# MircoWerner/VkRadixSort

Measured on AMD Instinct MI355X. Metric: Gkeys/s sorting 10^8 uint32 at 1/2/4/8 MI355X; % of HBM roofline, higher is better.
Workload: dtype u32

## Files before the change

vkradixsort_amd/csrc/vrs_device.hpp:

```cpp
#pragma once
#include "vrs_kernels.h"

#include <hip/hip_ext.h>

#include <type_traits>

#define VRS_LAUNCH(kernel, grid, block, stream, ev, ...)                                                        \
    do {                                                                                                        \
        if ((ev).start != nullptr || (ev).stop != nullptr)                                                      \
            hipExtLaunchKernelGGL(kernel, grid, block, 0, stream, (ev).start, (ev).stop, 0, __VA_ARGS__);       \
        else                                                                                                    \
            hipLaunchKernelGGL(kernel, grid, block, 0, stream, __VA_ARGS__);                                    \
    } while (0)

#ifndef VRS_MARK
#define VRS_MARK(i)
#define VRS_MARK_FLUSH(...)
#endif
namespace vrs {

constexpr size_t kStreamInBytes = size_t(128) << 20;

constexpr int kDtUnroll = 8;
constexpr int kLbItems = 16;
// ... 94 lines not shown
    for (int o = 1; o < 64; o <<= 1) {
        const uint32_t t = __shfl_up(incl, o);
        if (lane >= static_cast<uint32_t>(o)) incl += t;
    }
    if (lane == 63u) s_tmp[wave] = incl;
    __syncthreads();
    uint32_t base = 0;
#pragma unroll
    for (int j = 0; j < kWaves; ++j) base += (static_cast<uint32_t>(j) < wave) ? s_tmp[j] : 0u;
    return base + incl - v;
}

constexpr int RANK_BALLOT = 0;
constexpr int RANK_ATOMIC = 1;

template <typename K, int ITEMS, int WAVES, bool PAIRS = false>
struct ChunkSmem {
    K keys[ITEMS * WAVES * 64];
    uint32_t vals[PAIRS ? ITEMS * WAVES * 64 : 1];
    uint32_t whist[WAVES][kBins];
    uint32_t gbase[kBins];
    uint32_t scan_tmp[WAVES];
    uint32_t lb_gave_up;
};

__device__ __forceinline__ uint64_t match_any_digit(uint32_t d) {
    uint32_t lo = ~0u, hi = ~0u;
#pragma unroll
    for (int b = 0; b < 8; ++b) {
        const uint32_t m = static_cast<uint32_t>(__builtin_amdgcn_sbfe(static_cast<int>(d), b, 1));
        const uint64_t B = __builtin_amdgcn_uicmp(m, 0u, 33 );
        lo = __builtin_amdgcn_bitop3_b32(m, lo, static_cast<uint32_t>(B), 0x84);
        hi = __builtin_amdgcn_bitop3_b32(m, hi, static_cast<uint32_t>(B >> 32), 0x84);
    }
    return (static_cast<uint64_t>(hi) << 32) | lo;
}

template <int WAVES>
__device__ __forceinline__ uint32_t block_exclusive_scan_w(uint32_t v, uint32_t *s_tmp, uint32_t lane,
                                                           uint32_t wave) {
    uint32_t incl = v;
#pragma unroll
    for (int o = 1; o < 64; o <<= 1) {
        const uint32_t t = __shfl_up(incl, o);
        if (lane >= static_cast<uint32_t>(o)) incl += t;
    }
    if (lane == 63u) s_tmp[wave] = incl;
    __syncthreads();
    uint32_t base = 0;
#pragma unroll
    for (int j = 0; j < WAVES; ++j) base += (static_cast<uint32_t>(j) < wave) ? s_tmp[j] : 0u;
    return base + incl - v;
}

constexpr uint32_t kLbInclusive = 1u << 28, kLbValue = (1u << 28) - 1u, kLbTagShift = 29;

__device__ __forceinline__ uint32_t lb_load(const uint32_t *p) {
    return __hip_atomic_load(p, __ATOMIC_RELAXED, __HIP_MEMORY_SCOPE_AGENT);
}
__device__ __forceinline__ void lb_store_through(uint32_t *p, uint32_t v) {
    __hip_atomic_store(p, v, __ATOMIC_RELAXED, __HIP_MEMORY_SCOPE_AGENT);
}
__device__ __forceinline__ void lb_store_l2(uint32_t *p, uint32_t v) {
    __hip_atomic_store(p, v, __ATOMIC_RELAXED, __HIP_MEMORY_SCOPE_WORKGROUP);
}

struct NoLookback {
// ... 141 lines not shown
        }
        if constexpr (PAIRS) {
#pragma unroll
            for (int i = 0; i < ITEMS; ++i) {
                const uint32_t idx = seg + i * 64;
                val[i] = vin[FULL ? idx : (idx < valid ? idx : valid - 1u)];
            }
        }
    }
}
template <typename K, int ITEMS, typename DG>
__device__ __forceinline__ void chunk_pad(K (&key)[ITEMS], uint32_t valid, const DG &dg) {
    const uint32_t seg = (threadIdx.x >> 6) * (ITEMS * 64) + (threadIdx.x & 63u);
#pragma unroll
    for (int i = 0; i < ITEMS; ++i) key[i] = seg + i * 64 < valid ? key[i] : dg.template pad<K>();
}

template <typename K, int ITEMS, int WAVES, bool PAIRS, int RANK, bool FULL, typename DG, typename LB = NoLookback>
__device__ __forceinline__ void scatter_chunk_loaded(ChunkSmem<K, ITEMS, WAVES, PAIRS> &sm, K (&key)[ITEMS], uint32_t (&val)[PAIRS ? ITEMS : 1], K *kout,
                                                     uint32_t *vout, uint32_t valid, const DG &dg, uint32_t &run_off, const LB lb = {}) {
    constexpr uint32_t THREADS = WAVES * 64;
    const uint32_t tid = threadIdx.x;
    const uint32_t lane = tid & 63u;
    const uint32_t wave = tid >> 6;

    {
        uint32_t *z = &sm.whist[0][0];
#pragma unroll
        for (int v = 0; v < 4; ++v) z[v * THREADS + tid] = 0;
        if constexpr (LB::kEnabled) {
// ... 137 lines not shown

    if constexpr (PAIRS) {
#pragma unroll
        for (int i = 0; i < ITEMS; ++i) val[i] = sm.vals[i * THREADS + tid];
        if constexpr (LB::kPool) {
            lb.template store_values<ITEMS, THREADS, FULL>(val, dst, vout, valid);
        } else {
#pragma unroll
            for (int i = 0; i < ITEMS; ++i) {
                if (FULL || i * THREADS + tid < valid) vout[dst[i]] = val[i];
            }
        }
    }
}

template <typename K, int ITEMS, int WAVES, bool PAIRS, int RANK, bool FULL, typename DG, typename LB = NoLookback, typename SRC = NoPieces>
__device__ __forceinline__ void scatter_chunk(ChunkSmem<K, ITEMS, WAVES, PAIRS> &sm, const K *kin,
                                              const uint32_t *vin, K *kout, uint32_t *vout,
                                              uint32_t valid, const DG &dg, uint32_t &run_off, const LB lb = {},
                                              const SRC src = {}, bool stream_in = false) {
    VRS_MARK(0);
    K key[ITEMS];
    uint32_t val[PAIRS ? ITEMS : 1];
    if constexpr (SRC::kEnabled) {
        const uint32_t seg = (threadIdx.x >> 6) * (ITEMS * 64) + (threadIdx.x & 63u);
        uint32_t vs[ITEMS];
#pragma unroll
        for (int i = 0; i < ITEMS; ++i) vs[i] = src.first_slot;
#pragma unroll 1
        for (uint32_t p = src.p0; p < src.p1; ++p) {
            const uint32_t lo = __builtin_amdgcn_readlane(src.lo, p), len = __builtin_amdgcn_readlane(src.len, p), vd = __builtin_amdgcn_readlane(src.slot, p);
#pragma unroll
            for (int i = 0; i < ITEMS; ++i) {
                const uint32_t idx = seg + i * 64;
                vs[i] = idx - lo < len ? vd + (idx - lo) : vs[i];
            }
        }
#pragma unroll
        for (int i = 0; i < ITEMS; ++i) {
            const K k = *src.at(vs[i]);
            key[i] = (FULL || seg + i * 64 < valid) ? k : dg.template pad<K>();
        }
        if constexpr (PAIRS) {
#pragma unroll
            for (int i = 0; i < ITEMS; ++i) val[i] = *src.val_at(vs[i]);
        }
    } else {
        chunk_load<K, ITEMS, PAIRS, FULL>(kin, vin, valid, stream_in, key, val);
        if constexpr (!FULL) chunk_pad(key, valid, dg);
    }
    scatter_chunk_loaded<K, ITEMS, WAVES, PAIRS, RANK, FULL, DG, LB>(sm, key, val, kout, vout, valid, dg, run_off, lb);
}

constexpr uint32_t kMsdBits = 14, kMsdBuckets = 1u << kMsdBits;
constexpr uint32_t kMsdMinShift = 13, kMsdMaxShift = 18;
constexpr uint32_t kMsdProbeWord = kMsdBuckets + 8u * 256u, kMsdOverWord = kMsdProbeWord + 1u;
constexpr uint32_t kMsdSubBits = kMsdBits - 8, kMsdSub = 1u << kMsdSubBits;

struct BitsDigit {
    uint32_t shift, mask, base;
    __device__ __forceinline__ uint32_t operator()(uint32_t key) const { return ((key - base) >> shift) & mask; }
// ... 7 lines not shown
```

vkradixsort_amd/csrc/vrs_local_sort.hpp:

```cpp
#pragma once
#include "vrs_device.hpp"

namespace vrs {

constexpr int kLeanRow = 512 + 64;
constexpr int kLeanMaxVec = 7;
template <bool STREAM>
__device__ __forceinline__ void store_sorted(uint4 *p, const uint4 &q) {
    if constexpr (STREAM) {
        typedef uint32_t u32x4 __attribute__((ext_vector_type(4)));
        const u32x4 v = {q.x, q.y, q.z, q.w};
        __builtin_nontemporal_store(v, reinterpret_cast<u32x4 *>(p));
    } else {
        *p = q;
    }
}

__device__ __forceinline__ void rows_in_order() { __builtin_amdgcn_sched_barrier(0); }
template <int STRIDE, int VEC>
__device__ __forceinline__ void load_rows(uint32_t (&k)[4 * VEC], const uint32_t *src, uint32_t words, uint32_t t) {
    const uint32_t nvec = (words + 3u) / 4u;
#pragma unroll
    for (int j = 0; j < VEC; ++j) {
        uint32_t v = j * STRIDE + t;
        if (j == VEC - 1) v = v < nvec ? v : nvec - 1u;
        const uint4 q = reinterpret_cast<const uint4 *>(src)[v];
        if (j + 1 < VEC) rows_in_order();
        k[4 * j] = q.x;
        k[4 * j + 1] = q.y;
        k[4 * j + 2] = q.z;
        k[4 * j + 3] = q.w;
    }
}

__device__ __forceinline__ uint32_t wave_inclusive_sum(uint32_t x) {
    x += __builtin_amdgcn_update_dpp(0u, x, 0x111, 0xf, 0xf, false);
    x += __builtin_amdgcn_update_dpp(0u, x, 0x112, 0xf, 0xf, false);
    x += __builtin_amdgcn_update_dpp(0u, x, 0x114, 0xf, 0xf, false);
    x += __builtin_amdgcn_update_dpp(0u, x, 0x118, 0xf, 0xf, false);
    x += __builtin_amdgcn_update_dpp(0u, x, 0x142, 0xa, 0xf, false);
    x += __builtin_amdgcn_update_dpp(0u, x, 0x143, 0xc, 0xf, false);
    return x;
}

__device__ __forceinline__ void pinned(uint32_t &x) { asm volatile("" : "+v"(x)); }

template <int WAVES>
__device__ __forceinline__ uint32_t waves_before(const uint32_t *s_tmp, uint32_t wave) {
    static_assert(WAVES % 4 == 0, "whole 16-byte vectors");
    uint4 t[WAVES / 4];
#pragma unroll
    for (int g = 0; g < WAVES / 4; ++g) t[g] = reinterpret_cast<const uint4 *>(s_tmp)[g];
    uint32_t sum = 0;
#pragma unroll
    for (int g = 0; g < WAVES / 4; ++g) {
        sum += (4u * g + 0u < wave) ? t[g].x : 0u;
        sum += (4u * g + 1u < wave) ? t[g].y : 0u;
        sum += (4u * g + 2u < wave) ? t[g].z : 0u;
        sum += (4u * g + 3u < wave) ? t[g].w : 0u;
    }
    return sum;
}

template <int THREADS, int VEC, bool GUARD, bool STREAM = false, bool ALIGNED_IN = false>
__device__ __forceinline__ void lean_sort_body(uint32_t (&k)[4 * VEC], uint32_t *abase, uint32_t mis, uint32_t n, uint32_t *s_keys,
                                               uint32_t *s_hist2, uint32_t *s_tmp, bool guard1, bool guard2, uint32_t mis_in) {
    constexpr int WAVES = THREADS / 64, ITEMS = 4 * VEC, PER = 512 / THREADS;
    const uint32_t tid = threadIdx.x, lane = tid & 63u, wave = tid >> 6;
    const uint32_t end = mis + n;
    const uint32_t nvec = (end + 3u) / 4u;
    uint32_t rank[ITEMS];
    uint32_t *s_hist = s_hist2 + WAVES * kLeanRow;
#pragma unroll
    for (int j = 0; j < VEC; ++j)
#pragma unroll
        for (int c = 0; c < 4; ++c) {
            uint32_t a = (k[4 * j + c] << 2) & 0x7FCu;
// ... 504 lines not shown
```

vkradixsort_amd/csrc/vrs_msd_pool.hip:

```cpp
#include "vrs_local_sort.hpp"

#include <algorithm>
#include <cmath>

namespace vrs {

namespace {

constexpr uint32_t kPoolMinShift = 13, kPoolMaxShift = 18;
constexpr float kPoolSigmas = 6.0f;

__global__ __launch_bounds__(256) void pool_sample_kernel(const uint32_t *__restrict__ keys, uint32_t n, uint32_t key_base,
                                                          PoolStreams ps, PoolPlan *__restrict__ pool, uint32_t top_bits) {
    constexpr int kPerWave = kPoolSampleTiles / 4;
    constexpr int kLoads = kPoolSampleKeys / 64;
    __shared__ uint32_t s_hist[2][256];
    __shared__ uint32_t s_or;
    const uint32_t tid = threadIdx.x, lane = tid & 63u, wave = tid >> 6;
    s_hist[0][tid] = 0;
    s_hist[1][tid] = 0;
    if (tid == 0) s_or = 0;
    const uint32_t t0 = blockIdx.x * kPoolSampleTiles;
    const uint32_t s0 = t0 / ps.tiles_per_stream;
    uint32_t k[kPerWave][kLoads];
// ... 104 lines not shown
    static constexpr bool kEnabled = true;
    static constexpr bool kReserves = true;
    static constexpr bool kPool = true;
    bool foreign = false;
    uint32_t recounted = 0;
    int index = 0;
    const void *stream_keys = nullptr;
    uint32_t done = 0;
    uint32_t seed = 0;
    uint32_t *cursor = nullptr;
    const uint32_t *region = nullptr;
    uint32_t pad_keys = 0;
    uint32_t n_virt = 0;
    uint32_t *overflow = nullptr;
    uint32_t overflow_last = 0;
    uint32_t *gbase2 = nullptr, *split = nullptr, *flags = nullptr;
    uint32_t *fail_word = nullptr;
    mutable uint32_t reserved = 0, cnt = 0, rb = 0, rc = 0, ob = 0, oc = 0;
    mutable bool reserved_yet = false;

    __device__ __forceinline__ void publish(uint32_t v) const {
        if (reserved_yet) return;
        reserved_yet = true;
        cnt = v - pad_keys;
        if (cnt) reserved = __hip_atomic_fetch_add(cursor, cnt, __ATOMIC_RELAXED, __HIP_MEMORY_SCOPE_WORKGROUP);
    }
    __device__ __forceinline__ void load_region() {
        rb = region[0];
        rc = region[8 * 256];
        ob = region[16 * 256];
        oc = region[24 * 256];
// ... 9 lines not shown
        if (end <= rc) {
            g = rb + reserved - excl;
        } else if (reserved >= rc) {
            bad = end - rc > oc;
            g = n_virt + ob + (reserved - rc) - excl;
            if (cnt) atomicOr(flags, 2u);
        } else {
            bad = end - rc > oc;
            sp = excl + (rc - reserved);
            g = rb + reserved - excl;
            g2 = n_virt + ob - sp;
            atomicOr(flags, 3u);
        }
        if (cnt && bad) __hip_atomic_fetch_or(fail_word, 1u, __ATOMIC_RELAXED, __HIP_MEMORY_SCOPE_AGENT);
        gbase[tid] = g;
        gbase2[tid] = g2;
        split[tid] = sp;
    }
    template <typename K, int ITEMS, uint32_t THREADS, bool FULL, typename DG>
    __device__ __forceinline__ void store(const uint32_t *, const K (&key)[ITEMS], uint32_t (&dst)[ITEMS], K *kout, uint32_t valid, const DG &dg) const {
        const uint32_t tid = threadIdx.x;
        const uint32_t f = *flags;
        if (f == 0u) {
#pragma unroll
            for (int i = 0; i < ITEMS; ++i)
                if (FULL || i * THREADS + tid < valid) kout[dst[i]] = key[i];
            return;
        }
        if (f & 1u) {
#pragma unroll
            for (int i = 0; i < ITEMS; ++i) {
                const uint32_t d = dg(key[i]);
                if (i * THREADS + tid >= split[d]) dst[i] = gbase2[d] + (i * THREADS + tid);
            }
        }
#pragma unroll
        for (int i = 0; i < ITEMS; ++i) {
            K *p = dst[i] < n_virt ? kout + dst[i] : overflow + min(dst[i] - n_virt, overflow_last);
            if (FULL || i * THREADS + tid < valid) *p = key[i];
        }
    }
    uint32_t *overflow_values = nullptr;
    template <int ITEMS, uint32_t THREADS, bool FULL>
    __device__ __forceinline__ void store_values(const uint32_t (&val)[ITEMS], const uint32_t (&dst)[ITEMS], uint32_t *vout, uint32_t valid) const {
        const uint32_t tid = threadIdx.x;
        if (*flags == 0u) {
#pragma unroll
            for (int i = 0; i < ITEMS; ++i)
// ... 19 lines not shown
        }
        StreamLookback::publish(v);
    }
    __device__ __forceinline__ void refuse() const { __hip_atomic_fetch_or(at.fail_word, 1u, __ATOMIC_RELAXED, __HIP_MEMORY_SCOPE_AGENT); }
    __device__ __forceinline__ void place(uint32_t *gbase, uint32_t tid, uint32_t before, uint32_t excl) const { at.place_run(gbase, tid, before, excl); }
    template <typename K, int ITEMS, uint32_t THREADS, bool FULL, typename DG>
    __device__ __forceinline__ void store(const uint32_t *g, const K (&key)[ITEMS], uint32_t (&dst)[ITEMS], K *kout, uint32_t valid, const DG &dg) const {
        at.template store<K, ITEMS, THREADS, FULL>(g, key, dst, kout, valid, dg);
    }
    template <int ITEMS, uint32_t THREADS, bool FULL>
    __device__ __forceinline__ void store_values(const uint32_t (&val)[ITEMS], const uint32_t (&dst)[ITEMS], uint32_t *vout, uint32_t valid) const {
        at.template store_values<ITEMS, THREADS, FULL>(val, dst, vout, valid);
    }
};

__device__ __forceinline__ uint32_t xcc_place(unsigned long long xcc_map) {
    const uint32_t my_xcc = xcc_id();
    uint32_t x = 8u;
#pragma unroll
    for (uint32_t q = 0; q < 8u; ++q)
        if (x == 8u && xcc_of(xcc_map, q) == my_xcc) x = q;
    return x;
}

__device__ __forceinline__ uint32_t plan_word(const uint32_t *p) {
    return *(const uint32_t __attribute__((address_space(4))) *)(p);
}
__device__ __forceinline__ uint2 plan_word(const uint2 *p) {
    typedef uint32_t pair_t __attribute__((ext_vector_type(2)));
    const pair_t v = *(const pair_t __attribute__((address_space(4))) *)(p);
    return make_uint2(v.x, v.y);
}

template <bool PAIRS, bool FULL>
__device__ __forceinline__ void pool_pass_a_tile(ChunkSmem<uint32_t, 16, 8, PAIRS> &sm, uint32_t *gbase2, uint32_t *split, uint32_t *flags, const uint32_t *kin,
                                                 const uint32_t *vin, const uint32_t *slice_keys, uint32_t *keys_out, uint32_t *overflow, uint32_t n,
                                                 uint32_t key_base, PoolPlan *pool, MsdPlan *msd, uint32_t s_out, uint32_t i, uint32_t done, uint32_t valid,
                                                 uint32_t armed, uint32_t shift, uint32_t overflow_capacity, uint32_t par, const PoolPayloads &pv, uint32_t top_bits) {
    const bool stream_in = static_cast<size_t>(n) * sizeof(uint32_t) >= kStreamInBytes;
    VRS_MARK(0);
    uint32_t key[16], val[PAIRS ? 16 : 1];
    chunk_load<uint32_t, 16, PAIRS, FULL>(kin, vin, valid, stream_in, key, val);
    const uint32_t d = threadIdx.x & 255u, row = s_out & 7u;
    PoolReserve at;
    at.region = &pool->base[row][d];
    at.load_region();
    asm volatile("" : : "s"(kin), "s"(vin), "s"(pool) : "memory");
    if (armed == 0u) return;
    if (s_out == 8u) {
        if (threadIdx.x == 0) __hip_atomic_fetch_or(&pool->fail[par], 1u, __ATOMIC_RELAXED, __HIP_MEMORY_SCOPE_AGENT);
        return;
    }
    if (threadIdx.x == 0) __hip_atomic_fetch_add(&pool->claim_a[s_out * kPoolMaxTilesA + i], 1u, __ATOMIC_RELAXED, __HIP_MEMORY_SCOPE_WORKGROUP);
    if (threadIdx.x == 0) *flags = 0;
    RadixDigit<uint32_t> dg;
    dg.shift = shift + (kMsdBits - top_bits);
    dg.base = key_base;
    if constexpr (!FULL) chunk_pad(key, valid, dg);
    at.cursor = &msd->cursor_a[s_out][d];
    at.pad_keys = d == dg(dg.template pad<uint32_t>()) ? kPoolTile - valid : 0u;
    at.n_virt = n;
    at.overflow = overflow;
    at.overflow_last = overflow_capacity - 1u;
    at.gbase2 = gbase2;
    at.split = split;
    at.flags = flags;
    at.fail_word = &pool->fail[par];
    uint32_t unused = 0;
    if constexpr (PAIRS) {
        at.overflow_values = pv.overflow_values;
        PoolLookback lb;
        lb.at = at;
        lb.stream_keys = slice_keys;
        lb.done = done;
        lb.col = pv.status + static_cast<size_t>(s_out) * kBins + d;
        lb.stride = static_cast<size_t>(8) * kBins;
        lb.index = static_cast<int>(i);
        lb.tag = 1u << kLbTagShift;
        lb.budget = pv.spin_budget;
        lb.hold = pv.hold_tile >= 0 && i == static_cast<uint32_t>(pv.hold_tile);
        scatter_chunk_loaded<uint32_t, 16, 8, true, RANK_ATOMIC, FULL>(sm, key, val, keys_out, pv.values_partner, valid, dg, unused, lb);
    } else {
        scatter_chunk_loaded<uint32_t, 16, 8, false, RANK_ATOMIC, FULL>(sm, key, val, keys_out, nullptr, valid, dg, unused, at);
    }
}

template <bool PAIRS>
__global__ __launch_bounds__(512, 4) void pool_pass_a_kernel(const uint32_t *__restrict__ keys_in, uint32_t *__restrict__ keys_out,
                                                             uint32_t *__restrict__ overflow, uint32_t n, uint32_t key_base,
                                                             PoolStreams ps, PoolPlan *__restrict__ pool, MsdPlan *__restrict__ msd,
                                                             unsigned long long xcc_map, int misplace, uint32_t overflow_capacity, uint32_t par,
                                                             PoolPayloads pv, uint32_t top_bits) {
    __shared__ ChunkSmem<uint32_t, 16, 8, PAIRS> sm;
    __shared__ uint32_t s_gbase2[kBins], s_split[kBins], s_flags;
    VRS_MARK(6);
    const uint32_t armed = plan_word(&pool->armed), shift = plan_word(&pool->shift);
    const uint32_t i = blockIdx.x >> 3;
    const uint32_t s_out = xcc_place(xcc_map);
    const uint32_t s_in = (s_out + (misplace ? (i & 1u) : 0u)) & 7u;
    const uint32_t len = ps.len[s_in];
    const uint32_t done = i * kPoolTile;
    const uint32_t valid = done < len ? min(kPoolTile, len - done) : 0u;
    const uint32_t *slice_keys = keys_in + ps.start[s_in];
    const uint32_t *vin = PAIRS ? pv.values_home + ps.start[s_in] + done : nullptr;
    if (valid == kPoolTile)
        pool_pass_a_tile<PAIRS, true>(sm, s_gbase2, s_split, &s_flags, slice_keys + done, vin, slice_keys, keys_out, overflow, n, key_base, pool, msd, s_out, i,
                                      done, valid, armed, shift, overflow_capacity, par, pv, top_bits);
    else if (valid != 0u)
        pool_pass_a_tile<PAIRS, false>(sm, s_gbase2, s_split, &s_flags, slice_keys + done, vin, slice_keys, keys_out, overflow, n, key_base, pool, msd, s_out, i,
                                       done, valid, armed, shift, overflow_capacity, par, pv, top_bits);
    else if (armed != 0u) {
        if (s_out == 8u) {
            if (threadIdx.x == 0) __hip_atomic_fetch_or(&pool->fail[par], 1u, __ATOMIC_RELAXED, __HIP_MEMORY_SCOPE_AGENT);
        } else if (threadIdx.x == 0)
            __hip_atomic_fetch_add(&pool->claim_a[s_out * kPoolMaxTilesA + i], 1u, __ATOMIC_RELAXED, __HIP_MEMORY_SCOPE_WORKGROUP);
    }
    VRS_MARK_FLUSH(1);
}

constexpr float kPoolR = 40.0f;
template <uint32_t SUB>
__device__ __forceinline__ uint32_t pool_space(uint32_t c) {
    if (c == 0u) return 0u;
    const float x = static_cast<float>(c), s = static_cast<float>(SUB);
// ... 217 lines not shown
            msd->ok = 0;
        }
    }
}

struct SlackReserve {
    static constexpr bool kEnabled = true;
    static constexpr bool kReserves = true;
    static constexpr bool kPool = true;
    bool foreign = false;
    uint32_t recounted = 0;
    int index = 0;
    const void *stream_keys = nullptr;
    uint32_t done = 0;
    uint32_t seed = 0;
    uint32_t *cursor = nullptr;
    uint32_t start = 0, next = 0;
    uint32_t local_cap = 0;
    uint32_t *max_bucket = nullptr;
    uint32_t dump = 0;
    uint32_t pad_keys = 0;
    uint32_t above = 0, key_base = 0;
    uint32_t *fail_word = nullptr;
    mutable uint32_t reserved = 0, cnt = 0;
    mutable bool reserved_yet = false;

    __device__ __forceinline__ void publish(uint32_t v) const {
        if (reserved_yet) return;
        reserved_yet = true;
        cnt = v - pad_keys;
        if (cnt) reserved = __hip_atomic_fetch_add(cursor, cnt, __ATOMIC_RELAXED, __HIP_MEMORY_SCOPE_WORKGROUP);
    }
    __device__ __forceinline__ void fetch(int, uint32_t (&)[kLbBatch]) const {}
    __device__ __forceinline__ uint32_t resolve(uint32_t (&)[kLbBatch], bool &) const { return reserved; }
    __device__ __forceinline__ void refuse() const {}
    __device__ __forceinline__ void place(uint32_t *gbase, uint32_t tid, uint32_t, uint32_t excl) const { place_run(gbase, tid, reserved, excl); }
    __device__ __forceinline__ void place_run(uint32_t *gbase, uint32_t tid, uint32_t reserved, uint32_t excl) const {
        const uint32_t end = reserved + cnt;
        const bool bad = cnt != 0u && end > next - start;
        if (bad) {
            __hip_atomic_fetch_or(fail_word, 1u, __ATOMIC_RELAXED, __HIP_MEMORY_SCOPE_AGENT);
        } else if (cnt != 0u && end > local_cap) {
            __hip_atomic_fetch_or(fail_word, 2u, __ATOMIC_RELAXED, __HIP_MEMORY_SCOPE_AGENT);
            __hip_atomic_fetch_max(max_bucket, end, __ATOMIC_RELAXED, __HIP_MEMORY_SCOPE_AGENT);
        }
        gbase[tid] = (bad ? dump : start + reserved) - excl;
// ... 15 lines not shown
    __device__ __forceinline__ void store_values(const uint32_t (&val)[ITEMS], const uint32_t (&dst)[ITEMS], uint32_t *vout, uint32_t valid) const {
        const uint32_t tid = threadIdx.x;
#pragma unroll
        for (int i = 0; i < ITEMS; ++i)
            if (FULL || i * THREADS + tid < valid) vout[dst[i]] = val[i];
    }
};

struct SlackLookback : StreamLookback {
    static constexpr bool kPool = true;
    SlackReserve at;
    __device__ __forceinline__ void publish(uint32_t v) const {
        if (!at.reserved_yet) {
            at.reserved_yet = true;
            at.cnt = v - at.pad_keys;
            if (at.cnt) __hip_atomic_fetch_add(at.cursor, at.cnt, __ATOMIC_RELAXED, __HIP_MEMORY_SCOPE_WORKGROUP);
        }
        StreamLookback::publish(v);
    }
    __device__ __forceinline__ void refuse() const { __hip_atomic_fetch_or(at.fail_word, 1u, __ATOMIC_RELAXED, __HIP_MEMORY_SCOPE_AGENT); }
    __device__ __forceinline__ void place(uint32_t *gbase, uint32_t tid, uint32_t before, uint32_t excl) const { at.place_run(gbase, tid, before, excl); }
    template <typename K, int ITEMS, uint32_t THREADS, bool FULL, typename DG>
    __device__ __forceinline__ void store(const uint32_t *g, const K (&key)[ITEMS], uint32_t (&dst)[ITEMS], K *kout, uint32_t valid, const DG &dg) const {
        at.template store<K, ITEMS, THREADS, FULL>(g, key, dst, kout, valid, dg);
    }
    template <int ITEMS, uint32_t THREADS, bool FULL>
    __device__ __forceinline__ void store_values(const uint32_t (&val)[ITEMS], const uint32_t (&dst)[ITEMS], uint32_t *vout, uint32_t valid) const {
        at.template store_values<ITEMS, THREADS, FULL>(val, dst, vout, valid);
    }
};

template <uint32_t SUBBITS, bool PAIRS>
__global__ __launch_bounds__(512, PAIRS ? 4 : 6) void pool_pass_b_kernel(const uint32_t *__restrict__ regions, const uint32_t *__restrict__ overflow,
                                                             uint32_t *__restrict__ slack, const MsdPlan *__restrict__ msd, PoolPlan *__restrict__ pool,
                                                             uint32_t n_virt, uint32_t key_base, uint32_t local_cap, uint32_t dump,
                                                             unsigned long long xcc_map, uint32_t stamp, uint32_t grouped, uint32_t par, PoolPayloads pv,
                                                             uint32_t top_bits) {
    __shared__ ChunkSmem<uint32_t, 16, 8, PAIRS> sm;
    VRS_MARK(6);
    const uint32_t x = xcc_place(xcc_map), xs = x & 7u, j = blockIdx.x >> 3;
    const uint32_t ok_a = plan_word(&pool->ok_a), tiles = plan_word(&pool->tiles_b[xs][32]);
    const uint2 entry = plan_word(&pool->tile_map[xs][j < kPoolMaxTilesB ? j : 0u]);
    const uint32_t total = plan_word(&pool->top_base[256]), shift = plan_word(&pool->shift);
    asm volatile("" : : "s"(ok_a), "s"(tiles), "s"(entry.x), "s"(entry.y), "s"(total), "s"(shift), "s"(regions), "s"(overflow), "s"(slack), "s"(n_virt), "s"(stamp),
                 "s"(top_bits), "s"(key_base), "s"(local_cap), "s"(dump), "s"(grouped), "s"(par)
                 : "memory");
    if (ok_a == 0u) return;
    if (x == 8u) {
        if (threadIdx.x == 0) __hip_atomic_fetch_or(&pool->fail[par], 1u, __ATOMIC_RELAXED, __HIP_MEMORY_SCOPE_AGENT);
        return;
    }
    uint32_t claimed = 0;
    if (threadIdx.x == 0) claimed = __hip_atomic_exchange(&pool->claim_b[j * 8u + x], stamp, __ATOMIC_RELAXED, __HIP_MEMORY_SCOPE_WORKGROUP);
    if (j >= tiles) return;
    const uint32_t a = entry.y & 255u, tile_lo = (entry.y >> 8) * kPoolTile;
    const bool one_piece = entry.x != kPoolTileGeneral;
    const bool stream_in = static_cast<size_t>(total) * sizeof(uint32_t) >= kStreamInBytes;
    constexpr uint32_t SUB = 1u << SUBBITS;
    const uint32_t d = threadIdx.x & 255u, b = a * SUB + min(d, SUB - 1u);
    const BitsDigit dg{shift + kMsdBits - top_bits - SUBBITS, SUB - 1u, key_base};
    SlackReserve at;
    auto set_up = [&](uint32_t valid) {
        at.cursor = &pool->sub_cursor[b];
        at.start = pool->sub_start[b];
        at.next = pool->sub_start[b + 1u];
        at.local_cap = local_cap;
        at.max_bucket = &pool->max_bucket;
        at.dump = dump;
        at.pad_keys = d == SUB - 1u ? kPoolTile - valid : 0u;
        at.above = grouped ? 0xFF000000u : (shift + kMsdBits < 32u ? ~0u << (shift + kMsdBits) : 0u);
        at.key_base = grouped ? key_base + (a << 24) : key_base;
        at.fail_word = &pool->fail[par];
        if (threadIdx.x == 0 && claimed == stamp) __hip_atomic_fetch_or(&pool->fail[par], 1u, __ATOMIC_RELAXED, __HIP_MEMORY_SCOPE_AGENT);
    };
    auto chain = [&](SlackLookback &lb) {
        lb.at = at;
        lb.col = pv.status + (static_cast<size_t>(j - (entry.y >> 8)) * 8u + x) * kBins + d;
        lb.stride = static_cast<size_t>(8) * kBins;
        lb.index = static_cast<int>(entry.y >> 8);
        lb.tag = 6u << kLbTagShift;
        lb.budget = pv.spin_budget;
    };
    uint32_t unused = 0;
    if (one_piece) {
        const uint32_t slot0 = entry.x;
        const uint32_t *kin = slot0 < n_virt ? regions + slot0 : overflow + (slot0 - n_virt);
        const uint32_t *vin = !PAIRS ? nullptr : slot0 < n_virt ? pv.values_partner + slot0 : pv.overflow_values + (slot0 - n_virt);
        VRS_MARK(0);
        uint32_t key[16], val[PAIRS ? 16 : 1];
        chunk_load<uint32_t, 16, PAIRS, true>(kin, vin, kPoolTile, stream_in, key, val);
        asm volatile("" : "+v"(claimed) : : "memory");
        set_up(kPoolTile);
        if constexpr (PAIRS) {
            SlackLookback lb;
            chain(lb);
            scatter_chunk_loaded<uint32_t, 16, 8, true, RANK_ATOMIC, true, BitsDigit, SlackLookback>(sm, key, val, slack, pv.slack_values, kPoolTile, dg, unused, lb);
        } else {
            scatter_chunk_loaded<uint32_t, 16, 8, false, RANK_ATOMIC, true, BitsDigit, SlackReserve>(sm, key, val, slack, nullptr, kPoolTile, dg, unused, at);
        }
        VRS_MARK_FLUSH(2);
        return;
    }
    const uint32_t lane = threadIdx.x & 63u;
    const uint2 pc = pool->pieces[a][lane & 15u];
    const uint32_t pend = pc.x, pslot = pc.y;
    const uint32_t before = __shfl_up(pend, 1);
    const uint32_t plo = lane == 0u ? 0u : before;
    const uint32_t plen = lane < 16u ? pend - plo : 0u;
    const uint32_t keys_a = __builtin_amdgcn_readlane(pend, 15);
    const uint32_t valid = min(kPoolTile, keys_a - tile_lo);
    const unsigned long long touch = __ballot(plen != 0u && plo < tile_lo + valid && pend > tile_lo);
    PieceSrc src;
    src.p0 = static_cast<uint32_t>(__builtin_ctzll(touch | (1ull << 63)));
    src.p1 = 64u - static_cast<uint32_t>(__builtin_clzll(touch | 1ull));
    src.lo = plo - tile_lo;
    src.len = plen;
    src.slot = pslot;
    src.regions = regions;
    src.overflow = overflow;
    src.n_virt = n_virt;
    src.first_slot = __builtin_amdgcn_readlane(pslot, src.p0) + (tile_lo - __builtin_amdgcn_readlane(plo, src.p0));
    set_up(valid);
    if constexpr (PAIRS) {
        src.vregions = pv.values_partner;
        src.voverflow = pv.overflow_values;
        SlackLookback lb;
        chain(lb);
        if (valid == kPoolTile)
            scatter_chunk<uint32_t, 16, 8, true, RANK_ATOMIC, true, BitsDigit, SlackLookback, PieceSrc>(sm, nullptr, nullptr, slack, pv.slack_values, valid, dg, unused, lb, src);
        else
            scatter_chunk<uint32_t, 16, 8, true, RANK_ATOMIC, false, BitsDigit, SlackLookback, PieceSrc>(sm, nullptr, nullptr, slack, pv.slack_values, valid, dg, unused, lb, src);
    } else {
        if (valid == kPoolTile)
            scatter_chunk<uint32_t, 16, 8, false, RANK_ATOMIC, true, BitsDigit, SlackReserve, PieceSrc>(sm, nullptr, nullptr, slack, nullptr, valid, dg, unused, at, src);
        else
            scatter_chunk<uint32_t, 16, 8, false, RANK_ATOMIC, false, BitsDigit, SlackReserve, PieceSrc>(sm, nullptr, nullptr, slack, nullptr, valid, dg, unused, at, src);
    }
    VRS_MARK_FLUSH(2);
}

}


hipError_t launch_pool_sample(hipStream_t stream, const PoolSampleArgs &a, LaunchEvents ev) {
    const uint32_t *keys = a.keys;
    const uint32_t n = a.form.n, key_base = a.form.key_base, overflow_capacity = a.overflow_capacity, par = a.form.par, top_bits = a.form.top_bits;
    const PoolStreams &ps = a.form.ps;
    PoolPlan *pool = a.form.pool;
    if (n == 0 || ps.tiles_per_stream < kPoolSampleTiles) return hipErrorInvalidValue;
    const uint32_t grid = (ps.tiles_total + kPoolSampleTiles - 1u) / kPoolSampleTiles;
    VRS_LAUNCH(pool_sample_kernel, dim3(grid), dim3(256), stream, ev, keys, n, key_base, ps, pool, top_bits);
// ... 89 lines not shown
```

Measured before the change: 202.8.

## Use unstable single-histogram scatter for keys-only MSD pool passes

For keys-only sorting, the pool pass A and B kernels now use a new unstable scatter. It ranks keys with a single shared LDS histogram and workgroup atomics, with a whole-wave fast path when all lanes share a digit, instead of per-wave histograms. This shrinks LDS, which allows raising launch bounds occupancy to 6 for keys-only pass A. The split and second-base tables are merged into one uint2 array, the store path reads keys straight from LDS in batches of four, and block scans use DPP. Padding keys are no longer counted for keys-only runs. The risk is more contention on the shared-histogram atomics and loss of stability, which keys-only sorting does not need.

Result: no change. 202.9, median of 4 (+0.0%).

```diff
diff --git a/vkradixsort_amd/csrc/vrs_device.hpp b/vkradixsort_amd/csrc/vrs_device.hpp
--- a/vkradixsort_amd/csrc/vrs_device.hpp
+++ b/vkradixsort_amd/csrc/vrs_device.hpp
@@ -132,13 +132,13 @@
 constexpr int RANK_BALLOT = 0;
 constexpr int RANK_ATOMIC = 1;
 
-template <typename K, int ITEMS, int WAVES, bool PAIRS = false>
+template <typename K, int ITEMS, int WAVES, bool PAIRS = false, int TABLES = WAVES>
 struct ChunkSmem {
     K keys[ITEMS * WAVES * 64];
     uint32_t vals[PAIRS ? ITEMS * WAVES * 64 : 1];
-    uint32_t whist[WAVES][kBins];
+    uint32_t whist[TABLES][kBins];
     uint32_t gbase[kBins];
-    uint32_t scan_tmp[WAVES];
+    alignas(16) uint32_t scan_tmp[WAVES];
     uint32_t lb_gave_up;
 };
 
@@ -154,21 +154,40 @@
     return (static_cast<uint64_t>(hi) << 32) | lo;
 }
 
+__device__ __forceinline__ uint32_t wave_inclusive_sum(uint32_t x) {
+    x += __builtin_amdgcn_update_dpp(0u, x, 0x111, 0xf, 0xf, false);
+    x += __builtin_amdgcn_update_dpp(0u, x, 0x112, 0xf, 0xf, false);
+    x += __builtin_amdgcn_update_dpp(0u, x, 0x114, 0xf, 0xf, false);
+    x += __builtin_amdgcn_update_dpp(0u, x, 0x118, 0xf, 0xf, false);
+    x += __builtin_amdgcn_update_dpp(0u, x, 0x142, 0xa, 0xf, false);
+    x += __builtin_amdgcn_update_dpp(0u, x, 0x143, 0xc, 0xf, false);
+    return x;
+}
+
+template <int WAVES>
+__device__ __forceinline__ uint32_t waves_before(const uint32_t *s_tmp, uint32_t wave) {
+    static_assert(WAVES % 4 == 0, "whole 16-byte vectors");
+    uint4 t[WAVES / 4];
+#pragma unroll
+    for (int g = 0; g < WAVES / 4; ++g) t[g] = reinterpret_cast<const uint4 *>(s_tmp)[g];
+    uint32_t sum = 0;
+#pragma unroll
+    for (int g = 0; g < WAVES / 4; ++g) {
+        sum += (4u * g + 0u < wave) ? t[g].x : 0u;
+        sum += (4u * g + 1u < wave) ? t[g].y : 0u;
+        sum += (4u * g + 2u < wave) ? t[g].z : 0u;
+        sum += (4u * g + 3u < wave) ? t[g].w : 0u;
+    }
+    return sum;
+}
+
 template <int WAVES>
 __device__ __forceinline__ uint32_t block_exclusive_scan_w(uint32_t v, uint32_t *s_tmp, uint32_t lane,
                                                            uint32_t wave) {
-    uint32_t incl = v;
-#pragma unroll
-    for (int o = 1; o < 64; o <<= 1) {
-        const uint32_t t = __shfl_up(incl, o);
-        if (lane >= static_cast<uint32_t>(o)) incl += t;
-    }
+    const uint32_t incl = wave_inclusive_sum(v);
     if (lane == 63u) s_tmp[wave] = incl;
     __syncthreads();
-    uint32_t base = 0;
-#pragma unroll
-    for (int j = 0; j < WAVES; ++j) base += (static_cast<uint32_t>(j) < wave) ? s_tmp[j] : 0u;
-    return base + incl - v;
+    return waves_before<WAVES>(s_tmp, wave) + incl - v;
 }
 
 constexpr uint32_t kLbInclusive = 1u << 28, kLbValue = (1u << 28) - 1u, kLbTagShift = 29;
@@ -340,6 +359,31 @@
     const uint32_t seg = (threadIdx.x >> 6) * (ITEMS * 64) + (threadIdx.x & 63u);
 #pragma unroll
     for (int i = 0; i < ITEMS; ++i) key[i] = seg + i * 64 < valid ? key[i] : dg.template pad<K>();
+}
+template <typename K, int ITEMS, bool PAIRS, bool FULL, typename DG, typename SRC>
+__device__ __forceinline__ void chunk_load_pieces(const SRC &src, uint32_t valid, const DG &dg, K (&key)[ITEMS], uint32_t (&val)[PAIRS ? ITEMS : 1]) {
+    const uint32_t seg = (threadIdx.x >> 6) * (ITEMS * 64) + (threadIdx.x & 63u);
+    uint32_t vs[ITEMS];
+#pragma unroll
+    for (int i = 0; i < ITEMS; ++i) vs[i] = src.first_slot;
+#pragma unroll 1
+    for (uint32_t p = src.p0; p < src.p1; ++p) {
+        const uint32_t lo = __builtin_amdgcn_readlane(src.lo, p), len = __builtin_amdgcn_readlane(src.len, p), vd = __builtin_amdgcn_readlane(src.slot, p);
+#pragma unroll
+        for (int i = 0; i < ITEMS; ++i) {
+            const uint32_t idx = seg + i * 64;
+            vs[i] = idx - lo < len ? vd + (idx - lo) : vs[i];
+        }
+    }
+#pragma unroll
+    for (int i = 0; i < ITEMS; ++i) {
+        const K k = *src.at(vs[i]);
+        key[i] = (FULL || seg + i * 64 < valid) ? k : dg.template pad<K>();
+    }
+    if constexpr (PAIRS) {
+#pragma unroll
+        for (int i = 0; i < ITEMS; ++i) val[i] = *src.val_at(vs[i]);
+    }
 }
 
 template <typename K, int ITEMS, int WAVES, bool PAIRS, int RANK, bool FULL, typename DG, typename LB = NoLookback>
@@ -507,6 +551,87 @@
     }
 }
 
+template <typename K, int ITEMS, int WAVES, bool FULL, typename DG, typename LB>
+__device__ __forceinline__ void scatter_chunk_loaded_unstable(ChunkSmem<K, ITEMS, WAVES, false, 1> &sm, K (&key)[ITEMS], K *kout, uint32_t valid, const DG &dg,
+                                                              uint32_t bins, const LB lb) {
+    static_assert(LB::kReserves && LB::kPool && WAVES >= 4, "a reserving source of the pool form; the bins' waves' totals are one 16-byte read");
+    constexpr uint32_t THREADS = WAVES * 64;
+    const uint32_t tid = threadIdx.x;
+    const uint32_t lane = tid & 63u;
+    const uint32_t wave = tid >> 6;
+    uint32_t *hist = sm.whist[0];
+
+    if (tid < kBins) hist[tid] = 0;
+    __syncthreads();
+    VRS_MARK(1);
+
+    uint32_t rank[ITEMS];
+    if constexpr (!FULL) {
+        const uint32_t seg = wave * (ITEMS * 64) + lane;
+#pragma unroll
+        for (int i = 0; i < ITEMS; ++i) {
+            rank[i] = 0;
+            if (seg + i * 64 < valid) rank[i] = __hip_atomic_fetch_add(&hist[dg(key[i])], 1u, __ATOMIC_RELAXED, __HIP_MEMORY_SCOPE_WORKGROUP);
+        }
+    } else {
+#pragma unroll
+        for (int i = 0; i < ITEMS; ++i) {
+            const uint32_t d = dg(key[i]);
+            const uint32_t d0 = __builtin_amdgcn_readfirstlane(d);
+            if (__ballot(d == d0) == ~0ull) {
+                uint32_t old = 0;
+                if (lane == 0u) old = __hip_atomic_fetch_add(&hist[d0], 64u, __ATOMIC_RELAXED, __HIP_MEMORY_SCOPE_WORKGROUP);
+                rank[i] = __builtin_amdgcn_readfirstlane(old) + lane;
+            } else
+                rank[i] = __hip_atomic_fetch_add(&hist[d], 1u, __ATOMIC_RELAXED, __HIP_MEMORY_SCOPE_WORKGROUP);
+        }
+    }
+    __syncthreads();
+    VRS_MARK(2);
+
+    const bool owns = wave * 64u < bins;
+    const uint32_t total = opaque(hist[tid & (kBins - 1)]);
+    uint32_t incl = 0, excl = 0;
+    if (owns) {
+        incl = wave_inclusive_sum(total);
+        if (lane == 63u) sm.scan_tmp[wave] = incl;
+        lb.publish(total);
+    }
+    __syncthreads();
+    if (owns) {
+        excl = incl - total + waves_before<4>(sm.scan_tmp, wave);
+        hist[tid] = excl;
+    }
+    __syncthreads();
+    VRS_MARK(3);
+
+    static_assert(sizeof(K) == 4, "opaque() takes 32-bit keys");
+#pragma unroll
+    for (int i = 0; i < ITEMS; ++i) rank[i] += hist[dg(static_cast<K>(opaque(key[i])))];
+    if constexpr (!FULL) {
+        const uint32_t seg = wave * (ITEMS * 64) + lane;
+#pragma unroll
+        for (int i = 0; i < ITEMS; ++i) rank[i] = seg + i * 64 < valid ? rank[i] : seg + i * 64;
+    }
+#pragma unroll
+    for (int i = 0; i < ITEMS; ++i) sm.keys[rank[i]] = key[i];
+    if (owns) {
+        bool unused = false;
+        uint32_t none[kLbBatch];
+        lb.place(sm.gbase, tid, lb.resolve(none, unused), excl);
+    }
+    __syncthreads();
+    VRS_MARK(4);
+
+#pragma unroll
+    for (int i = 0; i < ITEMS; ++i) key[i] = sm.keys[i * THREADS + tid];
+    uint32_t dst[ITEMS];
+#pragma unroll
+    for (int i = 0; i < ITEMS; ++i) dst[i] = sm.gbase[dg(key[i])] + (i * THREADS + tid);
+    lb.template store<K, ITEMS, THREADS, FULL>(sm.gbase, key, dst, kout, valid, dg);
+    VRS_MARK(5);
+}
+
 template <typename K, int ITEMS, int WAVES, bool PAIRS, int RANK, bool FULL, typename DG, typename LB = NoLookback, typename SRC = NoPieces>
 __device__ __forceinline__ void scatter_chunk(ChunkSmem<K, ITEMS, WAVES, PAIRS> &sm, const K *kin,
                                               const uint32_t *vin, K *kout, uint32_t *vout,
@@ -516,28 +641,7 @@
     K key[ITEMS];
     uint32_t val[PAIRS ? ITEMS : 1];
     if constexpr (SRC::kEnabled) {
-        const uint32_t seg = (threadIdx.x >> 6) * (ITEMS * 64) + (threadIdx.x & 63u);
-        uint32_t vs[ITEMS];
-#pragma unroll
-        for (int i = 0; i < ITEMS; ++i) vs[i] = src.first_slot;
-#pragma unroll 1
-        for (uint32_t p = src.p0; p < src.p1; ++p) {
-            const uint32_t lo = __builtin_amdgcn_readlane(src.lo, p), len = __builtin_amdgcn_readlane(src.len, p), vd = __builtin_amdgcn_readlane(src.slot, p);
-#pragma unroll
-            for (int i = 0; i < ITEMS; ++i) {
-                const uint32_t idx = seg + i * 64;
-                vs[i] = idx - lo < len ? vd + (idx - lo) : vs[i];
-            }
-        }
-#pragma unroll
-        for (int i = 0; i < ITEMS; ++i) {
-            const K k = *src.at(vs[i]);
-            key[i] = (FULL || seg + i * 64 < valid) ? k : dg.template pad<K>();
-        }
-        if constexpr (PAIRS) {
-#pragma unroll
-            for (int i = 0; i < ITEMS; ++i) val[i] = *src.val_at(vs[i]);
-        }
+        chunk_load_pieces<K, ITEMS, PAIRS, FULL>(src, valid, dg, key, val);
     } else {
         chunk_load<K, ITEMS, PAIRS, FULL>(kin, vin, valid, stream_in, key, val);
         if constexpr (!FULL) chunk_pad(key, valid, dg);
diff --git a/vkradixsort_amd/csrc/vrs_local_sort.hpp b/vkradixsort_amd/csrc/vrs_local_sort.hpp
--- a/vkradixsort_amd/csrc/vrs_local_sort.hpp
+++ b/vkradixsort_amd/csrc/vrs_local_sort.hpp
@@ -33,34 +33,8 @@
     }
 }
 
-__device__ __forceinline__ uint32_t wave_inclusive_sum(uint32_t x) {
-    x += __builtin_amdgcn_update_dpp(0u, x, 0x111, 0xf, 0xf, false);
-    x += __builtin_amdgcn_update_dpp(0u, x, 0x112, 0xf, 0xf, false);
-    x += __builtin_amdgcn_update_dpp(0u, x, 0x114, 0xf, 0xf, false);
-    x += __builtin_amdgcn_update_dpp(0u, x, 0x118, 0xf, 0xf, false);
-    x += __builtin_amdgcn_update_dpp(0u, x, 0x142, 0xa, 0xf, false);
-    x += __builtin_amdgcn_update_dpp(0u, x, 0x143, 0xc, 0xf, false);
-    return x;
-}
 
 __device__ __forceinline__ void pinned(uint32_t &x) { asm volatile("" : "+v"(x)); }
-
-template <int WAVES>
-__device__ __forceinline__ uint32_t waves_before(const uint32_t *s_tmp, uint32_t wave) {
-    static_assert(WAVES % 4 == 0, "whole 16-byte vectors");
-    uint4 t[WAVES / 4];
-#pragma unroll
-    for (int g = 0; g < WAVES / 4; ++g) t[g] = reinterpret_cast<const uint4 *>(s_tmp)[g];
-    uint32_t sum = 0;
-#pragma unroll
-    for (int g = 0; g < WAVES / 4; ++g) {
-        sum += (4u * g + 0u < wave) ? t[g].x : 0u;
-        sum += (4u * g + 1u < wave) ? t[g].y : 0u;
-        sum += (4u * g + 2u < wave) ? t[g].z : 0u;
-        sum += (4u * g + 3u < wave) ? t[g].w : 0u;
-    }
-    return sum;
-}
 
 template <int THREADS, int VEC, bool GUARD, bool STREAM = false, bool ALIGNED_IN = false>
 __device__ __forceinline__ void lean_sort_body(uint32_t (&k)[4 * VEC], uint32_t *abase, uint32_t mis, uint32_t n, uint32_t *s_keys,
diff --git a/vkradixsort_amd/csrc/vrs_msd_pool.hip b/vkradixsort_amd/csrc/vrs_msd_pool.hip
--- a/vkradixsort_amd/csrc/vrs_msd_pool.hip
+++ b/vkradixsort_amd/csrc/vrs_msd_pool.hip
@@ -142,7 +142,9 @@
     uint32_t n_virt = 0;
     uint32_t *overflow = nullptr;
     uint32_t overflow_last = 0;
-    uint32_t *gbase2 = nullptr, *split = nullptr, *flags = nullptr;
+    uint2 *cross = nullptr;
+    uint32_t *flags = nullptr;
+    const uint32_t *lds_keys = nullptr;
     uint32_t *fail_word = nullptr;
     mutable uint32_t reserved = 0, cnt = 0, rb = 0, rc = 0, ob = 0, oc = 0;
     mutable bool reserved_yet = false;
@@ -182,11 +184,10 @@
         }
         if (cnt && bad) __hip_atomic_fetch_or(fail_word, 1u, __ATOMIC_RELAXED, __HIP_MEMORY_SCOPE_AGENT);
         gbase[tid] = g;
-        gbase2[tid] = g2;
-        split[tid] = sp;
+        cross[tid] = make_uint2(sp, g2);
     }
     template <typename K, int ITEMS, uint32_t THREADS, bool FULL, typename DG>
-    __device__ __forceinline__ void store(const uint32_t *, const K (&key)[ITEMS], uint32_t (&dst)[ITEMS], K *kout, uint32_t valid, const DG &dg) const {
+    __device__ __forceinline__ void store(const uint32_t *gbase_, const K (&key)[ITEMS], uint32_t (&dst)[ITEMS], K *kout, uint32_t valid, const DG &dg) const {
         const uint32_t tid = threadIdx.x;
         const uint32_t f = *flags;
         if (f == 0u) {
@@ -195,11 +196,46 @@
                 if (FULL || i * THREADS + tid < valid) kout[dst[i]] = key[i];
             return;
         }
+        if (lds_keys != nullptr) {
+#pragma unroll 1
+            for (uint32_t p0 = tid; p0 < ITEMS * THREADS; p0 += 4u * THREADS) {
+                K k[4];
+                uint32_t g[4];
+                unsigned long long c[4];
+#pragma unroll
+                for (int i = 0; i < 4; ++i) k[i] = lds_keys[p0 + i * THREADS];
+#pragma unroll
+                for (int i = 0; i < 4; ++i) {
+                    const uint32_t d = dg(k[i]);
+                    g[i] = gbase_[d];
+                    c[i] = reinterpret_cast<const unsigned long long *>(cross)[d];
+                }
+#pragma unroll
+                for (int i = 0; i < 4; ++i) asm volatile("" : "+v"(c[i]));
+#pragma unroll
+                for (int i = 0; i < 4; ++i) {
+                    const uint32_t p = p0 + i * THREADS;
+                    const uint32_t to = p >= static_cast<uint32_t>(c[i]) ? static_cast<uint32_t>(c[i] >> 32) + p : g[i] + p;
+                    K *q = to < n_virt ? kout + to : overflow + min(to - n_virt, overflow_last);
+                    if (FULL || p < valid) *q = k[i];
+                }
+            }
+            return;
+        }
         if (f & 1u) {
-#pragma unroll
-            for (int i = 0; i < ITEMS; ++i) {
-                const uint32_t d = dg(key[i]);
-                if (i * THREADS + tid >= split[d]) dst[i] = gbase2[d] + (i * THREADS + tid);
+            static_assert(ITEMS % 4 == 0, "four keys at a time");
+#pragma unroll
+            for (int h = 0; h < ITEMS; h += 4) {
+                unsigned long long c[4];
+#pragma unroll
+                for (int i = 0; i < 4; ++i) c[i] = reinterpret_cast<const unsigned long long *>(cross)[dg(key[h + i])];
+#pragma unroll
+                for (int i = 0; i < 4; ++i) asm volatile("" : "+v"(c[i]));
+#pragma unroll
+                for (int i = 0; i < 4; ++i) {
+                    const uint32_t p = (h + i) * THREADS + tid;
+                    dst[h + i] = p >= static_cast<uint32_t>(c[i]) ? static_cast<uint32_t>(c[i] >> 32) + p : dst[h + i];
+                }
             }
         }
 #pragma unroll
@@ -249,6 +285,11 @@
     }
 };
 
+template <bool PAIRS>
+using PoolSmem = ChunkSmem<uint32_t, 16, 8, PAIRS, PAIRS ? 8 : 1>;
+template <uint32_t SUB>
+constexpr uint32_t kPoolBinsB = SUB < 64u ? 64u : SUB;
+
 __device__ __forceinline__ uint32_t xcc_place(unsigned long long xcc_map) {
     const uint32_t my_xcc = xcc_id();
     uint32_t x = 8u;
@@ -268,7 +309,7 @@
 }
 
 template <bool PAIRS, bool FULL>
-__device__ __forceinline__ void pool_pass_a_tile(ChunkSmem<uint32_t, 16, 8, PAIRS> &sm, uint32_t *gbase2, uint32_t *split, uint32_t *flags, const uint32_t *kin,
+__device__ __forceinline__ void pool_pass_a_tile(PoolSmem<PAIRS> &sm, uint2 *cross, uint32_t *flags, const uint32_t *kin,
                                                  const uint32_t *vin, const uint32_t *slice_keys, uint32_t *keys_out, uint32_t *overflow, uint32_t n,
                                                  uint32_t key_base, PoolPlan *pool, MsdPlan *msd, uint32_t s_out, uint32_t i, uint32_t done, uint32_t valid,
                                                  uint32_t armed, uint32_t shift, uint32_t overflow_capacity, uint32_t par, const PoolPayloads &pv, uint32_t top_bits) {
@@ -291,14 +332,13 @@
     RadixDigit<uint32_t> dg;
     dg.shift = shift + (kMsdBits - top_bits);
     dg.base = key_base;
-    if constexpr (!FULL) chunk_pad(key, valid, dg);
+    if constexpr (!FULL && PAIRS) chunk_pad(key, valid, dg);
     at.cursor = &msd->cursor_a[s_out][d];
-    at.pad_keys = d == dg(dg.template pad<uint32_t>()) ? kPoolTile - valid : 0u;
+    at.pad_keys = PAIRS && d == dg(dg.template pad<uint32_t>()) ? kPoolTile - valid : 0u;
     at.n_virt = n;
     at.overflow = overflow;
     at.overflow_last = overflow_capacity - 1u;
-    at.gbase2 = gbase2;
-    at.split = split;
+    at.cross = cross;
     at.flags = flags;
     at.fail_word = &pool->fail[par];
     uint32_t unused = 0;
@@ -316,18 +356,20 @@
         lb.hold = pv.hold_tile >= 0 && i == static_cast<uint32_t>(pv.hold_tile);
         scatter_chunk_loaded<uint32_t, 16, 8, true, RANK_ATOMIC, FULL>(sm, key, val, keys_out, pv.values_partner, valid, dg, unused, lb);
     } else {
-        scatter_chunk_loaded<uint32_t, 16, 8, false, RANK_ATOMIC, FULL>(sm, key, val, keys_out, nullptr, valid, dg, unused, at);
+        at.lds_keys = sm.keys;
+        scatter_chunk_loaded_unstable<uint32_t, 16, 8, FULL>(sm, key, keys_out, valid, dg, 256u, at);
     }
 }
 
 template <bool PAIRS>
-__global__ __launch_bounds__(512, 4) void pool_pass_a_kernel(const uint32_t *__restrict__ keys_in, uint32_t *__restrict__ keys_out,
+__global__ __launch_bounds__(512, PAIRS ? 4 : 6) void pool_pass_a_kernel(const uint32_t *__restrict__ keys_in, uint32_t *__restrict__ keys_out,
                                                              uint32_t *__restrict__ overflow, uint32_t n, uint32_t key_base,
                                                              PoolStreams ps, PoolPlan *__restrict__ pool, MsdPlan *__restrict__ msd,
                                                              unsigned long long xcc_map, int misplace, uint32_t overflow_capacity, uint32_t par,
                                                              PoolPayloads pv, uint32_t top_bits) {
-    __shared__ ChunkSmem<uint32_t, 16, 8, PAIRS> sm;
-    __shared__ uint32_t s_gbase2[kBins], s_split[kBins], s_flags;
+    __shared__ PoolSmem<PAIRS> sm;
+    __shared__ uint2 s_cross[kBins];
+    __shared__ uint32_t s_flags;
     VRS_MARK(6);
     const uint32_t armed = plan_word(&pool->armed), shift = plan_word(&pool->shift);
     const uint32_t i = blockIdx.x >> 3;
@@ -339,10 +381,10 @@
     const uint32_t *slice_keys = keys_in + ps.start[s_in];
     const uint32_t *vin = PAIRS ? pv.values_home + ps.start[s_in] + done : nullptr;
     if (valid == kPoolTile)
-        pool_pass_a_tile<PAIRS, true>(sm, s_gbase2, s_split, &s_flags, slice_keys + done, vin, slice_keys, keys_out, overflow, n, key_base, pool, msd, s_out, i,
+        pool_pass_a_tile<PAIRS, true>(sm, s_cross, &s_flags, slice_keys + done, vin, slice_keys, keys_out, overflow, n, key_base, pool, msd, s_out, i,
                                       done, valid, armed, shift, overflow_capacity, par, pv, top_bits);
     else if (valid != 0u)
-        pool_pass_a_tile<PAIRS, false>(sm, s_gbase2, s_split, &s_flags, slice_keys + done, vin, slice_keys, keys_out, overflow, n, key_base, pool, msd, s_out, i,
+        pool_pass_a_tile<PAIRS, false>(sm, s_cross, &s_flags, slice_keys + done, vin, slice_keys, keys_out, overflow, n, key_base, pool, msd, s_out, i,
                                        done, valid, armed, shift, overflow_capacity, par, pv, top_bits);
     else if (armed != 0u) {
         if (s_out == 8u) {
@@ -590,7 +632,8 @@
     const void *stream_keys = nullptr;
     uint32_t done = 0;
     uint32_t seed = 0;
-    uint32_t *cursor = nullptr;
+    uint32_t *cursors = nullptr;
+    uint32_t bucket = 0;
     uint32_t start = 0, next = 0;
     uint32_t local_cap = 0;
     uint32_t *max_bucket = nullptr;
@@ -605,7 +648,7 @@
         if (reserved_yet) return;
         reserved_yet = true;
         cnt = v - pad_keys;
-        if (cnt) reserved = __hip_atomic_fetch_add(cursor, cnt, __ATOMIC_RELAXED, __HIP_MEMORY_SCOPE_WORKGROUP);
+        if (cnt) reserved = __hip_atomic_fetch_add(cursors + bucket, cnt, __ATOMIC_RELAXED, __HIP_MEMORY_SCOPE_WORKGROUP);
     }
     __device__ __forceinline__ void fetch(int, uint32_t (&)[kLbBatch]) const {}
     __device__ __forceinline__ uint32_t resolve(uint32_t (&)[kLbBatch], bool &) const { return reserved; }
@@ -651,7 +694,7 @@
         if (!at.reserved_yet) {
             at.reserved_yet = true;
             at.cnt = v - at.pad_keys;
-            if (at.cnt) __hip_atomic_fetch_add(at.cursor, at.cnt, __ATOMIC_RELAXED, __HIP_MEMORY_SCOPE_WORKGROUP);
+            if (at.cnt) __hip_atomic_fetch_add(at.cursors + at.bucket, at.cnt, __ATOMIC_RELAXED, __HIP_MEMORY_SCOPE_WORKGROUP);
         }
         StreamLookback::publish(v);
     }
@@ -673,7 +716,7 @@
                                                              uint32_t n_virt, uint32_t key_base, uint32_t local_cap, uint32_t dump,
                                                              unsigned long long xcc_map, uint32_t stamp, uint32_t grouped, uint32_t par, PoolPayloads pv,
                                                              uint32_t top_bits) {
-    __shared__ ChunkSmem<uint32_t, 16, 8, PAIRS> sm;
+    __shared__ PoolSmem<PAIRS> sm;
     VRS_MARK(6);
     const uint32_t x = xcc_place(xcc_map), xs = x & 7u, j = blockIdx.x >> 3;
     const uint32_t ok_a = plan_word(&pool->ok_a), tiles = plan_word(&pool->tiles_b[xs][32]);
@@ -698,13 +741,14 @@
     const BitsDigit dg{shift + kMsdBits - top_bits - SUBBITS, SUB - 1u, key_base};
     SlackReserve at;
     auto set_up = [&](uint32_t valid) {
-        at.cursor = &pool->sub_cursor[b];
+        at.cursors = pool->sub_cursor;
+        at.bucket = b;
         at.start = pool->sub_start[b];
         at.next = pool->sub_start[b + 1u];
         at.local_cap = local_cap;
         at.max_bucket = &pool->max_bucket;
         at.dump = dump;
-        at.pad_keys = d == SUB - 1u ? kPoolTile - valid : 0u;
+        at.pad_keys = PAIRS && d == SUB - 1u ? kPoolTile - valid : 0u;
         at.above = grouped ? 0xFF000000u : (shift + kMsdBits < 32u ? ~0u << (shift + kMsdBits) : 0u);
         at.key_base = grouped ? key_base + (a << 24) : key_base;
         at.fail_word = &pool->fail[par];
@@ -733,7 +777,7 @@
             chain(lb);
             scatter_chunk_loaded<uint32_t, 16, 8, true, RANK_ATOMIC, true, BitsDigit, SlackLookback>(sm, key, val, slack, pv.slack_values, kPoolTile, dg, unused, lb);
         } else {
-            scatter_chunk_loaded<uint32_t, 16, 8, false, RANK_ATOMIC, true, BitsDigit, SlackReserve>(sm, key, val, slack, nullptr, kPoolTile, dg, unused, at);
+            scatter_chunk_loaded_unstable<uint32_t, 16, 8, true>(sm, key, slack, kPoolTile, dg, kPoolBinsB<SUB>, at);
         }
         VRS_MARK_FLUSH(2);
         return;
@@ -741,8 +785,7 @@
     const uint32_t lane = threadIdx.x & 63u;
     const uint2 pc = pool->pieces[a][lane & 15u];
     const uint32_t pend = pc.x, pslot = pc.y;
-    const uint32_t before = __shfl_up(pend, 1);
-    const uint32_t plo = lane == 0u ? 0u : before;
+    const uint32_t plo = __builtin_amdgcn_update_dpp(0u, pend, 0x111, 0xf, 0xf, false);
     const uint32_t plen = lane < 16u ? pend - plo : 0u;
     const uint32_t keys_a = __builtin_amdgcn_readlane(pend, 15);
     const uint32_t valid = min(kPoolTile, keys_a - tile_lo);
@@ -757,8 +800,8 @@
     src.overflow = overflow;
     src.n_virt = n_virt;
     src.first_slot = __builtin_amdgcn_readlane(pslot, src.p0) + (tile_lo - __builtin_amdgcn_readlane(plo, src.p0));
-    set_up(valid);
     if constexpr (PAIRS) {
+        set_up(valid);
         src.vregions = pv.values_partner;
         src.voverflow = pv.overflow_values;
         SlackLookback lb;
@@ -768,10 +811,17 @@
         else
             scatter_chunk<uint32_t, 16, 8, true, RANK_ATOMIC, false, BitsDigit, SlackLookback, PieceSrc>(sm, nullptr, nullptr, slack, pv.slack_values, valid, dg, unused, lb, src);
     } else {
-        if (valid == kPoolTile)
-            scatter_chunk<uint32_t, 16, 8, false, RANK_ATOMIC, true, BitsDigit, SlackReserve, PieceSrc>(sm, nullptr, nullptr, slack, nullptr, valid, dg, unused, at, src);
-        else
-            scatter_chunk<uint32_t, 16, 8, false, RANK_ATOMIC, false, BitsDigit, SlackReserve, PieceSrc>(sm, nullptr, nullptr, slack, nullptr, valid, dg, unused, at, src);
+        VRS_MARK(0);
+        uint32_t key[16], val[1];
+        if (valid == kPoolTile) {
+            chunk_load_pieces<uint32_t, 16, false, true>(src, valid, dg, key, val);
+            set_up(valid);
+            scatter_chunk_loaded_unstable<uint32_t, 16, 8, true>(sm, key, slack, valid, dg, kPoolBinsB<SUB>, at);
+        } else {
+            chunk_load_pieces<uint32_t, 16, false, false>(src, valid, dg, key, val);
+            set_up(valid);
+            scatter_chunk_loaded_unstable<uint32_t, 16, 8, false>(sm, key, slack, valid, dg, kPoolBinsB<SUB>, at);
+        }
     }
     VRS_MARK_FLUSH(2);
 }
```
